# shenwei356/LexicMap

Measured on AMD Instinct MI355X. Metric: queries/sec (lexicmap search hot path, seed index HBM-resident), higher is better.
Workload: dtype u64

## Files before the change

### lexicmap_amd/csrc/lm_algos.h

```cpp
#pragma once
#include <stdint.h>

#if defined(__HIPCC__)
#define LM_HD __host__ __device__ __forceinline__
#define LM_HDN __host__ __device__ inline
#else
#define LM_HD inline
#define LM_HDN inline
#endif

#define LM_NULL_OFF (-1073741824)

LM_HD int lm_clz64(uint64_t x) {
#if defined(__HIP_DEVICE_COMPILE__)
    return x ? __clzll((long long)x) : 64;
#else
    return x ? __builtin_clzll(x) : 64;
#endif
}

LM_HD uint8_t lm_base2bit(uint8_t c) {
    switch (c | 0x20) {
    case 'c': case 'b': case 's': case 'y': return 1;
    case 'g': case 'k': return 2;
// ... 1165 lines not shown
    if ((key >> sh) & 3ull) return false;
    return lm_tree_search_miss(keys, n, key, p, K, lo, lo_out, hi_out);
}

#define LM_PFX_BASES 11
#define LM_PFX_BASES2 9
#define LM_PA_BLOOM_LOG_MAX 19
#define LM_PA_MAP9_LOG 18
LM_HD uint32_t lm_pa_filter_slot(uint32_t pfx, int log) {
    return (pfx * 0x9E3779B1u) >> (32 - log);
}
LM_HD int lm_pa_bloom_log(int log) { return log < LM_PA_BLOOM_LOG_MAX ? log : LM_PA_BLOOM_LOG_MAX; }
LM_HD uint32_t lm_mul24(uint32_t a, uint32_t b) {
#if defined(__HIP_DEVICE_COMPILE__)
    return __umul24(a, b);
#else
    return (uint32_t)((uint64_t)(a & 0xffffffu) * (uint64_t)(b & 0xffffffu));
#endif
}
LM_HD uint32_t lm_pa_bloom_slot(uint32_t pfx, int which, int blog) {
    return lm_mul24(pfx, which ? 0xB2AE35u : 0xEBCA6Bu) >> (32 - blog);
}
LM_HD uint64_t lm_pa_bits_words(int log) {
    return 2 * ((uint64_t)1 << (log - 5)) + ((uint64_t)1 << (lm_pa_bloom_log(log) - 5)) + ((uint64_t)1 << (LM_PA_MAP9_LOG - 5));
}
LM_HD int lm_pa_filter_log(int64_t nk) {
    int lg = 13;
    while (lg < 24 && ((int64_t)1 << lg) < 16 * nk) lg++;
    return lg;
}
#define LM_TAB_BITS_MIN 12
#define LM_TAB_BITS_MAX 20
LM_HD int lm_cmp_tab_bits(int64_t nk) {
    int tb = LM_TAB_BITS_MIN;
    while (tb < LM_TAB_BITS_MAX && ((int64_t)1 << tb) < 2 * nk) tb++;
    return tb;
}
LM_HD uint64_t lm_pa_bloom_word0(int log) { return 2 * ((uint64_t)1 << (log - 5)); }
LM_HD uint64_t lm_pa_map9_word0(int log) { return lm_pa_bloom_word0(log) + ((uint64_t)1 << (lm_pa_bloom_log(log) - 5)); }
template <typename OrBit> LM_HD void lm_pa_filter_set(uint64_t key, int K, int log, OrBit or_bit) {
    const uint32_t p11 = (uint32_t)(key >> ((K - LM_PFX_BASES) << 1)), p9 = (uint32_t)(key >> ((K - LM_PFX_BASES2) << 1));
    const int blog = lm_pa_bloom_log(log);
    const uint32_t h = lm_pa_filter_slot(p11, log), h2 = lm_pa_filter_slot(p9, log);
    or_bit((uint64_t)(h >> 5), 1u << (h & 31));
    or_bit(((uint64_t)1 << (log - 5)) + (h2 >> 5), 1u << (h2 & 31));
    const uint32_t a = lm_pa_bloom_slot(p11, 0, blog), b = lm_pa_bloom_slot(p11, 1, blog);
    or_bit(lm_pa_bloom_word0(log) + (a >> 5), 1u << (a & 31));
    or_bit(lm_pa_bloom_word0(log) + (b >> 5), 1u << (b & 31));
    or_bit(lm_pa_map9_word0(log) + (p9 >> 5), 1u << (p9 & 31));
}
LM_HD bool lm_pa_candidate(const uint32_t *bits, int log, uint64_t key, int p, int K) {
    const uint32_t h = lm_pa_filter_slot((uint32_t)(key >> ((K - LM_PFX_BASES) << 1)), log);
    if ((bits[h >> 5] >> (h & 31)) & 1u) return true;
    const uint64_t first_p = key >> ((K - p) << 1);
    if (first_p & ((1ull << ((p - 9) << 1)) - 1ull)) return false;
    if ((first_p & ((1ull << ((p - 7) << 1)) - 1ull)) == 0) return true;
    const uint32_t h2 = lm_pa_filter_slot((uint32_t)(key >> ((K - LM_PFX_BASES2) << 1)), log);
    const uint32_t *bits2 = bits + ((uint64_t)1 << (log - 5));
    return ((bits2[h2 >> 5] >> (h2 & 31)) & 1u) != 0;
}
LM_HD bool lm_pa_candidate2(const uint32_t *bloom, int blog, const uint32_t *map9, const uint32_t *bits11, int log,
                            uint32_t f, int p) {
    const uint32_t p11 = f >> ((p - LM_PFX_BASES) << 1);
    const uint32_t a = lm_pa_bloom_slot(p11, 0, blog), b = lm_pa_bloom_slot(p11, 1, blog);
    bool hit = (((bloom[a >> 5] >> (a & 31)) & (bloom[b >> 5] >> (b & 31))) & 1u) != 0;
    if (hit && log > blog) {
        const uint32_t h = lm_pa_filter_slot(p11, log);
        hit = ((bits11[h >> 5] >> (h & 31)) & 1u) != 0;
    }
    if (hit) return true;
    if (f & ((1u << ((p - 9) << 1)) - 1u)) return false;
    if ((f & ((1u << ((p - 7) << 1)) - 1u)) == 0) return true;
    const uint32_t p9 = f >> ((p - LM_PFX_BASES2) << 1);
    const bool m9 = ((map9[p9 >> 5] >> (p9 & 31)) & 1u) != 0;
    if (!m9) return false;
    if (p9 & 3u) {
        for (uint32_t sib = 1; sib < 4; sib++) {
            const uint32_t x = p11 | sib, sa = lm_pa_bloom_slot(x, 0, blog), sb = lm_pa_bloom_slot(x, 1, blog);
            bool h = (((bloom[sa >> 5] >> (sa & 31)) & (bloom[sb >> 5] >> (sb & 31))) & 1u) != 0;
            if (h && log > blog) {
                const uint32_t hh = lm_pa_filter_slot(x, log);
                h = ((bits11[hh >> 5] >> (hh & 31)) & 1u) != 0;
            }
            if (h) return true;
        }
        return false;
    }
    return true;
}

LM_HD bool lm_tree_search_range_tab(const uint64_t *keys, int n, uint64_t key, int p, int K, const uint32_t *tab,
                                    int tab_bits, int *lo_out, int *hi_out) {
    if (n <= 0) return false;
    if (p > K) p = K;
    const int sh = (K - p) << 1;
    const uint64_t low = sh >= 64 ? ~0ull : ((1ull << sh) - 1);
    const uint64_t left = key & ~low, right = key | low;
    const uint32_t b = (uint32_t)(key >> ((K << 1) - tab_bits));
    int lo = lm_lower_bound_u64(keys, (int)tab[b], (int)tab[b + 1], left);
    int hi = lm_upper_bound_u64(keys, lo, (int)tab[b + 1], right);
    if (lo < hi) {
        *lo_out = lo;
        *hi_out = hi;
        return true;
    }
    if ((key >> sh) & 3ull) return false;
    return lm_tree_search_miss(keys, n, key, p, K, lo, lo_out, hi_out);
}

LM_HD int lm_tree_search_first_tab(const uint64_t *keys, int n, uint64_t key, int p, int K, const uint32_t *tab, int tab_bits,
                                   int *lo_out, int *hi_out, uint64_t *right_out) {
// ... 434 lines not shown
```

### lexicmap_amd/csrc/lm_internal.h

```cpp
#pragma once
#include <hip/hip_runtime.h>

#include <algorithm>
#include <atomic>
#include <chrono>
#include <cstdio>
#include <cstdlib>
#include <map>
#include <memory>
#include <deque>
#include <mutex>
#include <shared_mutex>
#include <stdexcept>
#include <string>
#include <unordered_map>
#include <vector>

#include "../../include/lexicmap_hip.h"
#include "lm_format.h"
#include "lm_kernels.h"

namespace lm {

struct HipError : std::runtime_error {
// ... 372 lines not shown
    bool placing = false;
    void begin(lm_index *ix, int64_t local_genomes, int64_t max_genome_len);
    void count(const uint16_t *mask, const uint64_t *kmer, const uint64_t *val, int64_t n);
    void end_count();
    void place(const uint16_t *mask, const uint64_t *kmer, const uint64_t *val, int64_t n);
    void finish();
};
void sp_dump_range(const lm_index *src, hipStream_t st, const std::vector<int64_t> &off, bool flat, int64_t s0, int64_t s1,
                   uint16_t *s_mask, uint64_t *s_kmer, uint64_t *s_val, const uint64_t *new_bg = nullptr,
                   unsigned long long *n_out = nullptr);
void lm_screen_capture(lm_index *ix, hipStream_t st, const uint8_t *d_ascii, const std::vector<int64_t> &src_off,
                       const std::vector<int32_t> &len, const std::vector<int32_t> &reg_off, const std::vector<int32_t> &reg_s,
                       const std::vector<int32_t> &reg_e, uint64_t *d_kmers);
}

#define LM_WFA_CLASSES 5
struct lm_tune {
    int wfa_first_nc[LM_WFA_CLASSES] = {2, 2, 4, 8, 8};
    int wfa_win[LM_WFA_CLASSES] = {0, 0, 1, 0, 1};
    int chain1_wave = 1;
    int pa_filter_roll = 1;
    int pa_seg_by_group = 1;
    int pa_drop_nested = 1;
    int wfa_resident_pct = 100;
    int arena_reserve_pct = 90;
    int two_lanes = 1;
    int lookup_flat = 1;
    int wfa_r16 = 1;
    int wfa_serial = 0;
    int no_pipeline = 0;
    lm_tune() {
        if (const char *e = getenv("LM_WFA_FIRST_NC")) {
            int v[LM_WFA_CLASSES];
            if (sscanf(e, "%d,%d,%d,%d,%d", &v[0], &v[1], &v[2], &v[3], &v[4]) == LM_WFA_CLASSES)
                for (int c = 0; c < LM_WFA_CLASSES; c++)
                    if (v[c] == 1 || v[c] == 2 || v[c] == 4 || v[c] == 8 || v[c] == 16) wfa_first_nc[c] = v[c];
        }
        if (const char *e = getenv("LM_WFA_WIN"))
            for (int c = 0; c < LM_WFA_CLASSES && e[c]; c++) wfa_win[c] = e[c] == '1';
        if (const char *e = getenv("LM_WFA_R16")) wfa_r16 = atoi(e) != 0;
        if (const char *e = getenv("LM_LOOKUP_FLAT")) lookup_flat = atoi(e) != 0;
        if (const char *e = getenv("LM_CHAIN1_WAVE")) chain1_wave = atoi(e) != 0;
        if (const char *e = getenv("LM_TWO_LANES")) two_lanes = atoi(e) != 0;
        if (const char *e = getenv("LM_ARENA_RESERVE_PCT")) arena_reserve_pct = std::max(0, std::min(100, atoi(e)));
        if (const char *e = getenv("LM_PA_FILTER_ROLL")) pa_filter_roll = atoi(e) != 0;
        if (const char *e = getenv("LM_PA_DROP_NESTED")) pa_drop_nested = atoi(e) != 0;
    }
};

struct lm_index {
    lm_tune tune;
    int active_lanes = 1;
    int budget_lanes = 1;
    std::mutex mu;
    HostIndex host;
    lm_options opt;
    int device = 0;
    std::string err;
    DBuf<uint64_t> d_masks, d_pk_keys, d_pk_vals, d_out_kmers, d_out_vals, d_g_bg;
    DBuf<uint32_t> d_part_tab, d_g_keep;
    DBuf<int32_t> d_pfx_first, d_g_len, d_g2local;
    DBuf<int64_t> d_md_off, d_out_off, d_g_off, d_batch_first;
    int64_t n_seeds = 0, n_seeds_outlier = 0, seed_bytes = 0;
    int64_t scratch_budget = 0;
    DBuf<uint8_t> d_gbits;
    DBuf<float> d_gap_lut;
    int gap_lut_n = 0;
    DevIndexView view;
    int64_t hbm_bytes = 0;
// ... 48 lines not shown
```

### lexicmap_amd/csrc/lm_kernels.h

```cpp
#pragma once
#include <hip/hip_runtime.h>
#include <stdint.h>

#include "lm_algos.h"
#include "lm_residency.h"

namespace lm {

struct DevIndexView {
    int K, M, mask_prefix;
    const uint64_t *masks;
    const int32_t *pfx_first;
    int part_bases;
    int P1;
    int key_bits;
    int gid_bits, pos_bits;
    const uint64_t *pk_keys;
    const uint64_t *pk_vals;
    const uint32_t *part_tab;
    const int64_t *md_off;
    const uint64_t *g_bg;
    const uint32_t *g_keep;
    const uint64_t *out_kmers;
    const uint64_t *out_vals;
// ... 83 lines not shown
                       float min_score, int32_t *ntask);
void launch_make_tasks(hipStream_t st, DevIndexView ix, const uint64_t *segA, const int64_t *seg_off, int nseg,
                       const LmSub *subs, const int32_t *chain_off_pool, const int32_t *chain_idx_pool,
                       const int32_t *ntask, const int64_t *task_off, const int64_t *qoff, int ext_len,
                       int32_t *order_scratch, Task *tasks);
void launch_task_wlen(hipStream_t st, const Task *tasks, int64_t ntasks, int32_t *wlen);
void launch_task_set_woff(hipStream_t st, Task *tasks, int64_t ntasks, const int64_t *woff);
void launch_extract_windows(hipStream_t st, DevIndexView ix, const Task *tasks, const TaskSrc *src, int64_t ntasks,
                            const int32_t *only, uint8_t *wbuf);
void launch_extract_windows_at(hipStream_t st, DevIndexView ix, const Task *tasks, const TaskSrc *src, const int32_t *idx,
                               const int64_t *dest, int64_t n, uint8_t *wbuf);
void launch_stage_genome_bits(hipStream_t st, const StageCmd *cmds, int64_t n);
void launch_build_cmp_tab(hipStream_t st, const uint64_t *keys_cmp, const int64_t *posoff, const int32_t *nvalid, int nq,
                          int K, const int64_t *tab_off, const int32_t *tab_bits, int64_t tab_words, uint32_t *tab);
void launch_sum_i32(hipStream_t st, const int32_t *v, int64_t n, unsigned long long *out);
void launch_build_cmp_bits(hipStream_t st, const uint64_t *keys_cmp, const int64_t *posoff, const int32_t *nvalid, int nq,
                           int K, const int64_t *bits_off, const int32_t *bits_log, uint32_t *bits);
#define LM_PA_MAX_SEGS 8192
#define LM_PA_RANGE_SEGS 16
#define LM_PA_GROUP 64
void launch_pa_filter(hipStream_t st, DevIndexView ix, const Task *tasks, const TaskSrc *src, int64_t ntasks, const uint8_t *wbuf,
                      const int64_t *posoff, const int32_t *nvalid, const uint32_t *cmp_bits, const int64_t *bits_off,
                      const int32_t *bits_log, int K, int min_prefix, unsigned long long *seg_count, int nseg, int64_t seg_cap,
                      uint64_t *cand, unsigned long long *group_counter, int ncu, int seg_by_group, bool roll = true);
void launch_pa_search(hipStream_t st, DevIndexView ix, const Task *tasks, const TaskSrc *src, const uint8_t *wbuf, const uint64_t *keys_cmp,
                      const uint32_t *vals_cmp, const int64_t *posoff, const int32_t *nvalid, const uint32_t *cmp_tab,
                      const int64_t *tab_off, const int32_t *tab_bits, int K, int min_prefix,
                      const unsigned long long *seg_count, int nseg, int64_t seg_cap, const uint64_t *cand,
                      unsigned long long *count, int64_t cap, uint64_t *outA, uint64_t *outB, int qbits, int tbits,
                      int xcd_map, bool drop_nested = true);
void launch_pa_task_off_sorted(hipStream_t st, const uint64_t *sortedA, int shift, int64_t total, int64_t ntasks,
                               int64_t *pa_off);
void launch_pa_chain(hipStream_t st, const uint64_t *B, const int64_t *pa_off, int64_t ntasks, int K, LmChain2Opt opt,
                     LmSub *subs, uint8_t *marks, uint64_t *msi, int32_t *stack, LmChain2 *out, int32_t *out_n,
                     int32_t *clr_n, int qbits, int tbits);
void launch_gather_chain2(hipStream_t st, const LmChain2 *in, const int64_t *pa_off, const int32_t *out_n,
                          const int64_t *res_off, int64_t ntasks, LmChain2 *out);
void launch_extend_count(hipStream_t st, const HspIn *hsps, int64_t n, const uint8_t *qseq, const int64_t *qoff,
                         const uint8_t *wbuf, int32_t *cap);
void launch_extend_wave_cap(hipStream_t st, const int32_t *cap, int64_t n, int32_t *wcap, int64_t nw);
int extend_grid_blocks(int64_t n);
void launch_extend(hipStream_t st, const HspIn *hsps, int64_t n, const uint8_t *qseq, const int64_t *qoff,
                   const uint8_t *wbuf, const int32_t *cap, const int64_t *woff, uint16_t *subs, int32_t *msi,
                   void *rows_pool, uint32_t *rstart_pool, HspExt *out);
int wfa_resident_blocks(int device, int seq_words, int nc, bool win, bool r16 = false);
bool wfa_r16_ok(int seq_words, int nc, bool win);
void launch_wfa(hipStream_t st, const WfaIn *in, int64_t n, const int32_t *todo, int64_t ntodo, int nblocks,
// ... 9 lines not shown
```

### lexicmap_amd/csrc/lm_kernels.hip

```cpp
#include <hip/hip_runtime.h>
#include <stdint.h>

#include <algorithm>

#include "lm_algos.h"
#include "lm_kernels.h"
#include "lm_lookup_dev.h"

namespace lm {

#define LDS_WAVE_SYNC()                                        \
    do {                                                       \
        __builtin_amdgcn_fence(__ATOMIC_RELEASE, "wavefront"); \
        __builtin_amdgcn_wave_barrier();                       \
        __builtin_amdgcn_fence(__ATOMIC_ACQUIRE, "wavefront"); \
    } while (0)

__device__ __forceinline__ int find_segment(const int64_t *off, int n, int64_t x) {
    int lo = 0, hi = n;
    while (lo < hi) {
        int mid = (lo + hi + 1) >> 1;
        if (off[mid] <= x)
            lo = mid;
        else
// ... 63 lines not shown
        const int q = find_segment(tab_off, nq, t);
        const int bits = tab_bits[q], nb = 1 << bits;
        const int b = (int)(t - tab_off[q]);
        const uint64_t *keys = keys_cmp + 2 * posoff[q];
        int n = nvalid[q];
        int lo = n;
        if (b < nb) {
            uint64_t target = (uint64_t)b << ((K << 1) - bits);
            lo = lm_lower_bound_u64(keys, 0, n, target);
        }
        tab[t] = (uint32_t)lo;
    }
}
__global__ __launch_bounds__(256) void k_build_cmp_bits(const uint64_t *__restrict__ keys_cmp,
                                                         const int64_t *__restrict__ posoff,
                                                         const int32_t *__restrict__ nvalid, int nq, int K,
                                                         const int64_t *__restrict__ bits_off,
                                                         const int32_t *__restrict__ bits_log, uint32_t *__restrict__ bits) {
    for (int q = blockIdx.x; q < nq; q += gridDim.x) {
        const uint64_t *keys = keys_cmp + 2 * posoff[q];
        const int n = nvalid[q];
        const int log = bits_log[q];
        uint32_t *b = bits + bits_off[q];
        for (int j = threadIdx.x; j < n; j += blockDim.x)
            lm_pa_filter_set(keys[j], K, log, [&](uint64_t w, uint32_t m) { atomicOr(&b[w], m); });
    }
}

__global__ void k_fill_u32(uint32_t *p, int64_t n, uint32_t v) {
    for (int64_t i = (int64_t)blockIdx.x * blockDim.x + threadIdx.x; i < n; i += (int64_t)gridDim.x * blockDim.x) p[i] = v;
}

__global__ void k_mask(const uint64_t *__restrict__ keys_all, const int64_t *__restrict__ posoff, int nq, int M, int K,
                       const uint64_t *__restrict__ masks, uint64_t *__restrict__ out_kmers,
                       int64_t *__restrict__ out_lo, int64_t *__restrict__ out_hi, uint32_t *__restrict__ first_mask) {
    int64_t total = (int64_t)nq * M;
    for (int64_t t = (int64_t)blockIdx.x * blockDim.x + threadIdx.x; t < total; t += (int64_t)gridDim.x * blockDim.x) {
        int q = (int)(t / M), m = (int)(t % M);
        int64_t base = 2 * posoff[q];
        int n = (int)(2 * (posoff[q + 1] - posoff[q]));
        uint64_t kmer = 0;
        int lo = 0, hi = 0;
        if (n > 0) {
            kmer = lm_xor_argmin(keys_all + base, n, masks[m], &lo, &hi);
            if (kmer != 0 && lm_low_complexity(kmer, K)) kmer = 0;
            if (kmer != 0) atomicMin(&first_mask[base + lo], (uint32_t)m);
// ... 791 lines not shown
#define PA_SLICE_ROLL 2048
__device__ __forceinline__ uint32_t pa_rc16(uint32_t x) {
    const uint32_t y = __builtin_bitreverse32(~x);
    return ((y >> 1) & 0x55555555u) | ((y & 0x55555555u) << 1);
}
__device__ __forceinline__ bool pa_partial_rule(bool q, bool c, uint32_t f, int p, int blog, const uint32_t *bloom, const uint32_t *map9) {
    const uint32_t p9 = f >> ((p - 9) << 1);
    const bool all7 = (f & ((1u << ((p - 7) << 1)) - 1u)) == 0;
    const bool m9 = q && ((map9[p9 >> 5] >> (p9 & 31)) & 1u) != 0;
    const bool need = m9 && !all7 && (p9 & 3u) != 0;
    bool r = q ? (all7 || (m9 && (p9 & 3u) == 0)) : c;
    if (__ballot(need) != 0ull && need) {
        const uint32_t p11 = f >> ((p - LM_PFX_BASES) << 1);
        bool any = false;
#pragma unroll
        for (uint32_t sib = 1; sib < 4; sib++) {
            const uint32_t x = p11 | sib, sa = lm_pa_bloom_slot(x, 0, blog), sb = lm_pa_bloom_slot(x, 1, blog);
            any = any || (((bloom[sa >> 5] >> (sa & 31)) & (bloom[sb >> 5] >> (sb & 31))) & 1u) != 0;
        }
        r = any;
    }
    return r;
}
template <bool ROLL, bool SRC>
__global__ __launch_bounds__(PA_THREADS) void k_pa_filter(DevIndexView ix, const Task *__restrict__ tasks,
                                                           const TaskSrc *__restrict__ src, int64_t ntasks,
                                                           const uint8_t *__restrict__ wbuf,
                                                           const int64_t *__restrict__ posoff,
                                                           const int32_t *__restrict__ nvalid,
                                                           const uint32_t *__restrict__ cmp_bits,
                                                           const int64_t *__restrict__ bits_off,
                                                           const int32_t *__restrict__ bits_log, int K, int min_prefix,
                                                           unsigned long long *__restrict__ seg_count, int nseg,
                                                           int64_t seg_cap, uint64_t *__restrict__ cand,
                                                           unsigned long long *__restrict__ group_counter, int seg_by_group) {
    extern __shared__ uint64_t pa_lds[];
    uint64_t *s_stage = pa_lds;
    uint32_t *s_bloom = (uint32_t *)(pa_lds + PA_WAVES * PA_STAGE);
    uint32_t *s_map9 = s_bloom + (1 << (LM_PA_BLOOM_LOG_MAX - 5));
    uint64_t *s_pend_rec = (uint64_t *)(s_map9 + (1 << (LM_PA_MAP9_LOG - 5)));
    uint32_t *s_pend_pf = (uint32_t *)(s_pend_rec + PA_WAVES * PA_PEND);
    const int tid = threadIdx.x, lane = tid & 63, wave = tid >> 6;
    uint64_t *stg = s_stage + wave * PA_STAGE;
    int n_stg = 0;
    const uint64_t lt_mask = lane ? (~0ull >> (64 - lane)) : 0ull;
    int seg = (int)(((int64_t)blockIdx.x * PA_WAVES + wave) % nseg);
    uint64_t *seg_list = cand + (int64_t)seg * seg_cap;
// ... 5 lines not shown
        for (int j = lane; j < n_stg; j += 64)
            if ((int64_t)(base + (unsigned long long)j) < seg_cap) seg_list[base + (unsigned long long)j] = stg[j];
        n_stg = 0;
    };
    auto push = [&](bool c, uint64_t rec) {
        const uint64_t m = __ballot(c);
        if (m == 0) return;
        if (c) stg[n_stg + __popcll(m & lt_mask)] = rec;
        n_stg += __popcll(m);
        if (n_stg > PA_STAGE - 128) flush();
    };
    uint32_t *pend_pf = s_pend_pf + wave * PA_PEND;
    uint64_t *pend_rec = s_pend_rec + wave * PA_PEND;
    int n_pend = 0;
    const uint32_t *cur_qbits = nullptr;
    int cur_log = 0, cur_blog = 0;
    auto pend_round = [&](int cnt) {
        const int idx = n_pend - cnt + lane;
        bool c = false;
        uint64_t rec = 0;
        if (lane < cnt) {
            const uint32_t e = pend_pf[idx];
            rec = pend_rec[idx];
            c = lm_pa_candidate2(s_bloom, cur_blog, s_map9, cur_qbits, cur_log, e & 0x3fffffffu, LM_PFX_BASES + 2 * (int)(e >> 30));
        }
        n_pend -= cnt;
        push(c, rec);
    };
    auto pend = [&](bool c, uint32_t e, uint64_t rec) {
        const uint64_t m = __ballot(c);
        if (m == 0) return;
        if (c) {
            const int slot = n_pend + __popcll(m & lt_mask);
            pend_pf[slot] = e;
            pend_rec[slot] = rec;
        }
        n_pend += __popcll(m);
        while (n_pend >= 64) pend_round(64);
    };
    __shared__ int32_t s_q[PA_GROUP], s_rc[PA_GROUP], s_tb[PA_GROUP], s_wlen[PA_GROUP], s_npos[PA_GROUP], s_log[PA_GROUP];
    __shared__ int32_t s_first[PA_GROUP + 1];
    __shared__ int64_t s_goff[PA_GROUP], s_bits[PA_GROUP], s_woff[PA_GROUP];
    __shared__ const uint8_t *s_gb[SRC ? PA_GROUP : 1];
    __shared__ int s_next;
    __shared__ unsigned long long s_grp;
    const int64_t ngroups = (ntasks + PA_GROUP - 1) / PA_GROUP;
    while (true) {
        __syncthreads();
        if (tid == 0) s_grp = atomicAdd(group_counter, 1ull);
        __syncthreads();
        const int64_t grp = (int64_t)s_grp;
        if (grp >= ngroups) break;
        const int64_t t0g = grp * PA_GROUP;
        const int ng = (int)((ntasks < t0g + PA_GROUP ? ntasks : t0g + PA_GROUP) - t0g);
        if (seg_by_group) {
            const int gseg = (int)(grp * (int64_t)(nseg / PA_WAVES) / ngroups) * PA_WAVES + wave;
            if (gseg != seg) {
                flush();
                seg = gseg;
                seg_list = cand + (int64_t)seg * seg_cap;
// ... 9 lines not shown
            s_wlen[tid] = t.wlen;
            s_npos[tid] = n > 0 && t.wlen - K + 1 > 0 ? t.wlen - K + 1 : 0;
            if constexpr (SRC) {
                s_gb[tid] = t.g >= 0 ? src[t0g + tid].base : nullptr;
                s_goff[tid] = t.g >= 0 ? src[t0g + tid].off : 0;
            } else {
                s_goff[tid] = t.g >= 0 ? ix.g_off[t.g] : -1;
            }
            s_woff[tid] = t.woff;
            s_bits[tid] = cmp_bits ? bits_off[t.q] : -1;
            s_log[tid] = cmp_bits ? bits_log[t.q] : 0;
        }
        __syncthreads();
        int r0 = 0;
        while (r0 < ng) {
            int r1 = r0 + 1;
            while (r1 < ng && s_q[r1] == s_q[r0]) r1++;
            const int log = s_log[r0], blog = lm_pa_bloom_log(log);
            const uint32_t *qbits = s_bits[r0] >= 0 ? cmp_bits + s_bits[r0] : nullptr;
            cur_qbits = qbits;
            cur_log = log;
            cur_blog = blog;
            if (qbits != nullptr && K >= 16) {
                const uint32_t *gbl = qbits + lm_pa_bloom_word0(log), *g9 = qbits + lm_pa_map9_word0(log);
                const int nb = 1 << (blog - 5);
                for (int j = tid; j < nb; j += PA_THREADS) s_bloom[j] = gbl[j];
                for (int j = tid; j < (1 << (LM_PA_MAP9_LOG - 5)); j += PA_THREADS) s_map9[j] = g9[j];
            }
            if (tid == 0) {
                int acc = 0;
                for (int j = r0; j < r1; j++) {
                    s_first[j] = acc;
                    acc += (s_npos[j] + (ROLL ? PA_SLICE_ROLL : PA_SLICE) - 1) / (ROLL ? PA_SLICE_ROLL : PA_SLICE);
                }
                s_first[r1] = acc;
                s_next = 0;
            }
            __syncthreads();
            const int nslices = s_first[r1];
            while (true) {
                int sl = 0;
                if (lane == 0) sl = atomicAdd(&s_next, 1);
                sl = __builtin_amdgcn_readfirstlane(sl);
                if (sl >= nslices) break;
                int lo = r0, hi = r1;
                while (hi - lo > 1) {
                    const int mid = (lo + hi) >> 1;
// ... 46 lines not shown
#pragma unroll 1
                    for (int half = 0; half < 2; half++) {
#pragma unroll
                        for (int jj = 0; jj < 16; jj++) {
                            if (16 * half + jj >= bpl) break;
                            const int sh = 2 * jj;
                            const uint32_t xw = sh ? __builtin_amdgcn_alignbit(S0, S1, 32 - sh) : S0;
                            const int orc = 66 - 2 * jj;
                            const uint32_t Ra = (orc >> 5) == 2 ? R2 : R1, Rb = (orc >> 5) == 2 ? R3 : R2;
                            const uint32_t yw = (orc & 31) ? __builtin_amdgcn_alignbit(Ra, Rb, 32 - (orc & 31)) : Ra;
                            const uint32_t first = xw >> shp, rl = yw >> shp;
                            const uint32_t pf0 = t.rc ? rl : first, pf1 = t.rc ? first : rl;
                            const int r = rl0 + 16 * half + jj;
                            const int i = t.rc ? p1 - 1 - r : p0 + r;
                            const bool in = r < np;
                            bool c0, c1;
                            const uint32_t a0 = pf0 >> sha, a1 = pf1 >> sha;
                            const uint32_t s00 = lm_pa_bloom_slot(a0, 0, blog), s01 = lm_pa_bloom_slot(a0, 1, blog);
                            const uint32_t s10 = lm_pa_bloom_slot(a1, 0, blog), s11 = lm_pa_bloom_slot(a1, 1, blog);
                            const uint32_t b00 = s_bloom[s00 >> 5], b01 = s_bloom[s01 >> 5];
                            const uint32_t b10 = s_bloom[s10 >> 5], b11 = s_bloom[s11 >> 5];
                            const bool h0 = in && (((b00 >> (s00 & 31)) & (b01 >> (s01 & 31))) & 1u) != 0;
                            const bool h1 = in && (((b10 >> (s10 & 31)) & (b11 >> (s11 & 31))) & 1u) != 0;
                            const bool q0 = in && !h0 && (pf0 & m9p) == 0, q1 = in && !h1 && (pf1 & m9p) == 0;
                            c0 = h0;
                            c1 = h1;
                            if (log > blog) {
                                c0 = c1 = false;
                                const uint64_t rec = rec_t | ((uint64_t)(uint32_t)i << 1);
                                pend(h0 || q0, pf0 | pcode, rec);
                                pend(h1 || q1, pf1 | pcode, rec | 1ull);
                            } else if (__ballot(q0 || q1) != 0ull) {
                                c0 = pa_partial_rule(q0, c0, pf0, p, blog, s_bloom, s_map9);
                                c1 = pa_partial_rule(q1, c1, pf1, p, blog, s_bloom, s_map9);
                            }
                            const uint64_t m0 = __ballot(c0), m1 = __ballot(c1);
                            if ((m0 | m1) != 0ull) {
                                const int n0 = __popcll(m0);
                                const uint64_t rec = rec_t | ((uint64_t)(uint32_t)i << 1);
                                if (c0) stg[n_stg + __popcll(m0 & lt_mask)] = rec;
                                if (c1) stg[n_stg + n0 + __popcll(m1 & lt_mask)] = rec | 1ull;
                                n_stg += n0 + __popcll(m1);
                                if (n_stg > PA_STAGE - 128) flush();
                            }
                        }
                        S0 = S1;
                        S1 = S2;
                        R3 = R2;
                        R2 = R1;
                        R1 = R0;
                    }
                } else if (fast_pfx) {
                    const int np = p1 - p0;
                    const int g0 = t.rc ? t.tBegin + t.wlen - K - (p1 - 1) : t.tBegin + p0;
                    const int64_t abs0 = goff * 4 + g0;
                    const int64_t w0 = abs0 >> 5;
                    const int nwords = (int)(((abs0 + np + K - 2) >> 5) - w0) + 2;
                    const int lw = lane < nwords ? lane : nwords - 1;
                    const uint64_t Wl = __builtin_bswap64(((const uint64_t *)gb)[w0 + lw]);
                    for (int tile = 0; tile < np; tile += 64) {
                        const int r = tile + lane;
                        const int64_t ab = abs0 + r;
                        const int wi = (int)((ab >> 5) - w0), o = (int)(ab & 31) * 2;
                        const uint64_t H = __shfl(Wl, wi, 64), L = __shfl(Wl, wi + 1, 64);
                        const uint64_t v = o ? ((H << o) | (L >> (64 - o))) : H;
                        const uint32_t first = (uint32_t)(v >> (64 - 2 * p));
                        const uint32_t last = (uint32_t)(v >> (64 - 2 * K)) & ((1u << (2 * p)) - 1u);
                        const uint32_t rl = revcomp_small(last, p);
                        const uint32_t pf0 = t.rc ? rl : first, pf1 = t.rc ? first : rl;
                        const int i = t.rc ? p1 - 1 - r : p0 + r;
                        const bool in = r < np;
                        bool c0, c1;
                        {
                            const uint32_t a0 = pf0 >> ((p - LM_PFX_BASES) << 1), a1 = pf1 >> ((p - LM_PFX_BASES) << 1);
                            const uint32_t s00 = lm_pa_bloom_slot(a0, 0, blog), s01 = lm_pa_bloom_slot(a0, 1, blog);
                            const uint32_t s10 = lm_pa_bloom_slot(a1, 0, blog), s11 = lm_pa_bloom_slot(a1, 1, blog);
                            const uint32_t b00 = s_bloom[s00 >> 5], b01 = s_bloom[s01 >> 5];
                            const uint32_t b10 = s_bloom[s10 >> 5], b11 = s_bloom[s11 >> 5];
                            const bool h0 = in && (((b00 >> (s00 & 31)) & (b01 >> (s01 & 31))) & 1u) != 0;
                            const bool h1 = in && (((b10 >> (s10 & 31)) & (b11 >> (s11 & 31))) & 1u) != 0;
                            const uint32_t m9p = (1u << ((p - 9) << 1)) - 1u;
                            const bool q0 = in && !h0 && (pf0 & m9p) == 0, q1 = in && !h1 && (pf1 & m9p) == 0;
                            c0 = h0;
                            c1 = h1;
                            if (log > blog) {
                                c0 = c1 = false;
                                const uint64_t rec = rec_t | ((uint64_t)(uint32_t)i << 1);
                                const uint32_t pcode = (uint32_t)((p - LM_PFX_BASES) >> 1) << 30;
                                pend(h0 || q0, pf0 | pcode, rec);
                                pend(h1 || q1, pf1 | pcode, rec | 1ull);
                            } else if (__ballot(q0 || q1) != 0ull) {
                                c0 = pa_partial_rule(q0, c0, pf0, p, blog, s_bloom, s_map9);
                                c1 = pa_partial_rule(q1, c1, pf1, p, blog, s_bloom, s_map9);
                            }
                        }
                        const uint64_t m0 = __ballot(c0), m1 = __ballot(c1);
                        if ((m0 | m1) != 0ull) {
                            const int n0 = __popcll(m0);
                            const uint64_t rec = rec_t | ((uint64_t)(uint32_t)i << 1);
                            if (c0) stg[n_stg + __popcll(m0 & lt_mask)] = rec;
                            if (c1) stg[n_stg + n0 + __popcll(m1 & lt_mask)] = rec | 1ull;
                            n_stg += n0 + __popcll(m1);
                            if (n_stg > PA_STAGE - 128) flush();
                        }
                    }
                } else {
                    for (int tile = p0; tile < p1; tile += 64) {
                        const int i = tile + lane;
                        uint64_t kmer = 0, rc = 0;
                        if (i < p1) pa_kmer(t, w, gb, goff, i, K, &kmer, &rc);
#pragma unroll
                        for (int strand = 0; strand < 2; strand++) {
                            const bool c = i < p1 && (!use_bits || lm_pa_candidate(qbits, log, strand ? rc : kmer, p, K));
                            push(c, rec_t | ((uint64_t)(uint32_t)i << 1) | (uint64_t)strand);
                        }
                    }
// ... 1131 lines not shown
                               const int64_t *dest, int64_t n, uint8_t *wbuf) {
    if (n <= 0) return;
    hipLaunchKernelGGL(src ? k_extract_windows_at<true> : k_extract_windows_at<false>, dim3((unsigned)std::min<int64_t>(n, 65536)), dim3(256), 0, st, ix, tasks, src, idx, dest,
                       n, wbuf);
}
void launch_stage_genome_bits(hipStream_t st, const StageCmd *cmds, int64_t n) {
    if (n <= 0) return;
    hipLaunchKernelGGL(k_stage_genome_bits, dim3((unsigned)std::min<int64_t>(n, 65536)), dim3(256), 0, st, cmds, n);
}
void launch_build_cmp_tab(hipStream_t st, const uint64_t *keys_cmp, const int64_t *posoff, const int32_t *nvalid, int nq,
                          int K, const int64_t *tab_off, const int32_t *tab_bits, int64_t tab_words, uint32_t *tab) {
    LM_LAUNCH_1D(k_build_cmp_tab, tab_words, st, keys_cmp, posoff, nvalid, nq, K, tab_off, tab_bits, tab);
}
void launch_sum_i32(hipStream_t st, const int32_t *v, int64_t n, unsigned long long *out) {
    int g = (int)((n + 255) / 256);
    g = g < 1 ? 1 : (g > 2048 ? 2048 : g);
    hipLaunchKernelGGL(k_sum_i32, dim3(g), dim3(256), 0, st, v, n, out);
}
void launch_build_cmp_bits(hipStream_t st, const uint64_t *keys_cmp, const int64_t *posoff, const int32_t *nvalid, int nq,
                           int K, const int64_t *bits_off, const int32_t *bits_log, uint32_t *bits) {
    int g = nq < 1 ? 1 : (nq > 65536 ? 65536 : nq);
    hipLaunchKernelGGL(k_build_cmp_bits, dim3(g), dim3(256), 0, st, keys_cmp, posoff, nvalid, nq, K, bits_off, bits_log, bits);
}
void launch_pa_filter(hipStream_t st, DevIndexView ix, const Task *tasks, const TaskSrc *src, int64_t ntasks, const uint8_t *wbuf,
                      const int64_t *posoff, const int32_t *nvalid, const uint32_t *cmp_bits, const int64_t *bits_off,
                      const int32_t *bits_log, int K, int min_prefix, unsigned long long *seg_count, int nseg, int64_t seg_cap,
                      uint64_t *cand, unsigned long long *group_counter, int ncu, int seg_by_group, bool roll) {
    const int64_t ngroups = (ntasks + PA_GROUP - 1) / PA_GROUP;
    int g = (int)(ngroups < 1 ? 1 : (ngroups > ncu ? ncu : ngroups));
    static bool lds_set = false;
    if (!lds_set) {
        (void)hipFuncSetAttribute((const void *)k_pa_filter<true, false>, hipFuncAttributeMaxDynamicSharedMemorySize, PA_LDS_BYTES);
        (void)hipFuncSetAttribute((const void *)k_pa_filter<false, false>, hipFuncAttributeMaxDynamicSharedMemorySize, PA_LDS_BYTES);
        (void)hipFuncSetAttribute((const void *)k_pa_filter<true, true>, hipFuncAttributeMaxDynamicSharedMemorySize, PA_LDS_BYTES);
        (void)hipFuncSetAttribute((const void *)k_pa_filter<false, true>, hipFuncAttributeMaxDynamicSharedMemorySize, PA_LDS_BYTES);
        lds_set = true;
    }
    roll = roll && K == 31;
    auto kern = src ? (roll ? k_pa_filter<true, true> : k_pa_filter<false, true>) : (roll ? k_pa_filter<true, false> : k_pa_filter<false, false>);
    hipLaunchKernelGGL(kern, dim3(g), dim3(PA_THREADS), PA_LDS_BYTES, st, ix, tasks, src, ntasks, wbuf,
                       posoff, nvalid, cmp_bits, bits_off, bits_log, K, min_prefix, seg_count, nseg, seg_cap, cand, group_counter,
                       seg_by_group);
}
void launch_pa_search(hipStream_t st, DevIndexView ix, const Task *tasks, const TaskSrc *src, const uint8_t *wbuf, const uint64_t *keys_cmp,
                      const uint32_t *vals_cmp, const int64_t *posoff, const int32_t *nvalid, const uint32_t *cmp_tab,
                      const int64_t *tab_off, const int32_t *tab_bits, int K, int min_prefix,
                      const unsigned long long *seg_count, int nseg, int64_t seg_cap, const uint64_t *cand,
                      unsigned long long *count, int64_t cap, uint64_t *outA, uint64_t *outB, int qbits, int tbits,
                      int xcd_map, bool drop_nested) {
    int bps = xcd_map ? 256 / LM_PA_RANGE_SEGS : (256 * 32 + nseg - 1) / nseg;
    const int64_t need = (seg_cap + 255) / 256;
    if (bps > need) bps = (int)(need < 1 ? 1 : need);
    const int nseg8 = xcd_map ? (nseg / LM_PA_RANGE_SEGS + 7) / 8 * 8 * LM_PA_RANGE_SEGS : nseg;
    static const bool ps_dbg = getenv("LM_DEBUG_PA_SEARCH") != nullptr;
    static unsigned long long *d_dbg = nullptr;
    if (ps_dbg && !d_dbg && hipMalloc((void **)&d_dbg, 8 * sizeof(unsigned long long)) != hipSuccess) d_dbg = nullptr;
    if (ps_dbg && d_dbg) (void)hipMemsetAsync(d_dbg, 0, 8 * sizeof(unsigned long long), st);
    hipLaunchKernelGGL(src ? k_pa_search<true> : k_pa_search<false>, dim3(nseg8 * bps), dim3(256), 0, st, ix, tasks, src, wbuf, keys_cmp, vals_cmp, posoff, nvalid, cmp_tab,
                       tab_off, tab_bits, K, min_prefix, seg_count, seg_cap, bps, cand, count, cap, outA, outB, qbits, tbits, nseg,
                       xcd_map, drop_nested ? 1 : 0, ps_dbg ? d_dbg : nullptr);
    if (ps_dbg && d_dbg) {
        unsigned long long h[8] = {0};
// ... 95 lines not shown
```

### lexicmap_amd/csrc/lm_pipeline.hip

```cpp
#include <hip/hip_runtime.h>

#include <algorithm>
#include <chrono>
#include <cmath>
#include <cstdio>
#include <cstdlib>
#include <malloc.h>
#include <cstring>
#include <map>
#include <mutex>
#include <optional>
#include <sys/stat.h>
#include <stdexcept>
#include <tuple>
#include <string>
#include <unordered_map>
#include <vector>

#include "../../include/lexicmap_hip.h"
#include "lm_format.h"
#include "lm_kernels.h"

#include "lm_internal.h"
#include "lm_prims.h"
// ... 1502 lines not shown

extern "C" lm_status lm_qbatch_upload(lm_index *ix, const lm_query *queries, size_t nq, lm_qbatch **out) {
    *out = nullptr;
    if (!ix) return LM_ERR_ARG;
    if (nq >= ((size_t)1 << 31)) {
        ix->err = "query batch too large; split the batch";
        return LM_ERR_ARG;
    }
    try {
        std::lock_guard<std::mutex> lock(ix->mu);
        HIPCHK(hipSetDevice(ix->device));
        int64_t max_pos, max_qm;
        part_limits(ix, &max_pos, &max_qm);
        const int K = ix->host.k, M = ix->host.M;
        std::vector<size_t> cuts{0};
        int64_t pos = 0, nqp = 0;
        for (size_t i = 0; i < nq; i++) {
            const int64_t np = std::max<int64_t>((int64_t)queries[i].len - K + 1, 0);
            if (np > max_pos) {
                ix->err = "a query of " + std::to_string(queries[i].len) + " bases exceeds what one pass can hold (" +
                          std::to_string(max_pos) + " k-mers)";
                return LM_ERR_ARG;
            }
            if (nqp > 0 && (pos + np > max_pos || (nqp + 1) * (int64_t)M > max_qm)) {
                cuts.push_back(i);
                pos = 0;
                nqp = 0;
            }
            pos += np;
            nqp++;
        }
        cuts.push_back(nq);
        if (cuts.size() == 2) {
            *out = upload_part(ix, queries, nq, 0);
            return LM_OK;
        }
        lm_qbatch *top = new lm_qbatch();
        top->ix = ix;
        top->nq = (int)nq;
        try {
            for (size_t c = 0; c + 1 < cuts.size(); c++)
                top->parts.push_back(upload_part(ix, queries + cuts[c], cuts[c + 1] - cuts[c], (uint32_t)cuts[c]));
        } catch (...) {
            delete top;
            throw;
        }
        for (auto *p : top->parts) {
// ... 234 lines not shown
        for (int q = 0; q < qb->nq; q++) maxq = std::max<int64_t>(maxq, qb->h_qoff[q + 1] - qb->h_qoff[q]);
        if (maxq < 8192) by_group = false;
    }
    bool nseg_stale = false;
    for (int attempt = 0;; attempt++) {
        if (!compact) a.A0.ensure((size_t)a.pa_cap);
        a.B0.ensure((size_t)a.pa_cap);
        a.B1.ensure((size_t)a.pa_cap);
        if (!by_group) {
            if (attempt == 0 || nseg_stale) nseg = (int)std::max<int64_t>(1, std::min<int64_t>(1024, a.pa_cap / 4096));
            nseg_stale = false;
        } else if (attempt == 0) {
            const int64_t ngroups = (nt + LM_PA_GROUP - 1) / LM_PA_GROUP;
            const int64_t ranges = std::max<int64_t>(1, std::min<int64_t>(std::min<int64_t>(LM_PA_MAX_SEGS / LM_PA_RANGE_SEGS, ngroups),
                                                                          a.pa_cap / 4096 / LM_PA_RANGE_SEGS));
            nseg = (int)ranges * LM_PA_RANGE_SEGS;
        }
        const int64_t seg_cap = a.pa_cap / nseg;
        HIPCHK(hipMemsetAsync(a.pa_count.p, 0, (size_t)(2 + nseg) * sizeof(unsigned long long), S(ix)));
        {
            Prof p(ix, "k_pa_filter", W);
            launch_pa_filter(S(ix), ix->view, tasks_d, src_d, nt, a.wb, qb->posoff_cmp(), a.w->nvalid.p, a.w->cmp_bits.p,
                             qb->d_bits_off.p, qb->d_bits_log.p, LM_CMP_K, 11, a.pa_count.p + 2, nseg, seg_cap, a.B1.p,
                             a.pa_count.p + 1, device_cus(ix->device), by_group ? 1 : 0, ix->tune.pa_filter_roll != 0);
        }
        {
            Prof p(ix, "k_pa_search");
            launch_pa_search(S(ix), ix->view, tasks_d, src_d, a.wb, a.w->k_cmp, a.w->v_cmp, qb->posoff_cmp(), a.w->nvalid.p,
                             a.w->cmp_tab.p, qb->d_tab_off.p, qb->d_tab_bits.p, LM_CMP_K, 11, a.pa_count.p + 2, nseg, seg_cap,
                             a.B1.p, a.pa_count.p, a.pa_cap, a.A0.p, a.B0.p, compact ? qbits : 0, compact ? tbits : 0,
                             by_group ? 1 : 0, ix->tune.pa_drop_nested != 0);
        }
        std::vector<unsigned long long> hv((size_t)2 + nseg);
        HIPCHK(hipMemcpyAsync(hv.data(), a.pa_count.p, hv.size() * sizeof(unsigned long long), hipMemcpyDeviceToHost, S(ix)));
        sync(ix);
        TP = (int64_t)hv[0];
        int64_t ncand = 0, seg_max = 0;
        for (int j = 0; j < nseg; j++) {
            ncand += (int64_t)hv[2 + j];
            seg_max = std::max<int64_t>(seg_max, (int64_t)hv[2 + j]);
        }
        {
            int64_t idx = 0;
            uint32_t prevq = 0xffffffffu;
            for (int64_t i = 0; i < nt; i++)
                if (ht[i].q != prevq) {
                    prevq = ht[i].q;
// ... 2327 lines not shown
```

Measured before the change: 1377.

## Precompute partial-prefix rule bitmap per query to simplify prefix filter

Adds a second 9-base bitmap per query, built alongside the filter bits, that precomputes the partial-prefix acceptance rule (the sibling check over 11-mer prefixes). The prefix filter kernel gets a RULE template variant that tests this bit directly instead of running the sibling bloom loop, and only pends bloom hits that the rule does not already accept. A new pend2 helper batches both lanes with one ballot pass. The cost is more per-query bitmap memory (about 32 KB extra), a preset pass in the bit-build kernel, and query-batch splitting that now accounts for the larger bitmap, which may yield more batches.

```diff
diff --git a/lexicmap_amd/csrc/lm_algos.h b/lexicmap_amd/csrc/lm_algos.h
--- a/lexicmap_amd/csrc/lm_algos.h
+++ b/lexicmap_amd/csrc/lm_algos.h
@@ -1211,7 +1211,7 @@
     return lm_mul24(pfx, which ? 0xB2AE35u : 0xEBCA6Bu) >> (32 - blog);
 }
 LM_HD uint64_t lm_pa_bits_words(int log) {
-    return 2 * ((uint64_t)1 << (log - 5)) + ((uint64_t)1 << (lm_pa_bloom_log(log) - 5)) + ((uint64_t)1 << (LM_PA_MAP9_LOG - 5));
+    return 2 * ((uint64_t)1 << (log - 5)) + ((uint64_t)1 << (lm_pa_bloom_log(log) - 5)) + 2 * ((uint64_t)1 << (LM_PA_MAP9_LOG - 5));
 }
 LM_HD int lm_pa_filter_log(int64_t nk) {
     int lg = 13;
@@ -1227,6 +1227,10 @@
 }
 LM_HD uint64_t lm_pa_bloom_word0(int log) { return 2 * ((uint64_t)1 << (log - 5)); }
 LM_HD uint64_t lm_pa_map9_word0(int log) { return lm_pa_bloom_word0(log) + ((uint64_t)1 << (lm_pa_bloom_log(log) - 5)); }
+LM_HD uint64_t lm_pa_rule_word0(int log) { return lm_pa_map9_word0(log) + ((uint64_t)1 << (LM_PA_MAP9_LOG - 5)); }
+template <typename OrBit> LM_HD void lm_pa_filter_preset(int log, int j0, int step, OrBit or_bit) {
+    for (int j = j0; j < (1 << (LM_PA_MAP9_LOG - 5)); j += step) or_bit(lm_pa_rule_word0(log) + (uint64_t)j, 0x00010001u);
+}
 template <typename OrBit> LM_HD void lm_pa_filter_set(uint64_t key, int K, int log, OrBit or_bit) {
     const uint32_t p11 = (uint32_t)(key >> ((K - LM_PFX_BASES) << 1)), p9 = (uint32_t)(key >> ((K - LM_PFX_BASES2) << 1));
     const int blog = lm_pa_bloom_log(log);
@@ -1237,6 +1241,7 @@
     or_bit(lm_pa_bloom_word0(log) + (a >> 5), 1u << (a & 31));
     or_bit(lm_pa_bloom_word0(log) + (b >> 5), 1u << (b & 31));
     or_bit(lm_pa_map9_word0(log) + (p9 >> 5), 1u << (p9 & 31));
+    if ((p9 & 3u) == 0 || ((p11 & 0xfu) >= 1u && (p11 & 0xfu) <= 3u)) or_bit(lm_pa_rule_word0(log) + (p9 >> 5), 1u << (p9 & 31));
 }
 LM_HD bool lm_pa_candidate(const uint32_t *bits, int log, uint64_t key, int p, int K) {
     const uint32_t h = lm_pa_filter_slot((uint32_t)(key >> ((K - LM_PFX_BASES) << 1)), log);
@@ -1276,6 +1281,21 @@
         return false;
     }
     return true;
+}
+LM_HD bool lm_pa_rule_bit(const uint32_t *rule, uint32_t f, int p) {
+    const uint32_t p9 = f >> ((p - LM_PFX_BASES2) << 1);
+    return (f & ((1u << ((p - 9) << 1)) - 1u)) == 0 && ((rule[p9 >> 5] >> (p9 & 31)) & 1u) != 0;
+}
+LM_HD bool lm_pa_candidate3(const uint32_t *bloom, int blog, const uint32_t *rule, const uint32_t *bits11, int log,
+                            uint32_t f, int p) {
+    const uint32_t p11 = f >> ((p - LM_PFX_BASES) << 1);
+    const uint32_t a = lm_pa_bloom_slot(p11, 0, blog), b = lm_pa_bloom_slot(p11, 1, blog);
+    bool hit = (((bloom[a >> 5] >> (a & 31)) & (bloom[b >> 5] >> (b & 31))) & 1u) != 0;
+    if (hit && log > blog) {
+        const uint32_t h = lm_pa_filter_slot(p11, log);
+        hit = ((bits11[h >> 5] >> (h & 31)) & 1u) != 0;
+    }
+    return hit || lm_pa_rule_bit(rule, f, p);
 }
 
 LM_HD bool lm_tree_search_range_tab(const uint64_t *keys, int n, uint64_t key, int p, int K, const uint32_t *tab,
diff --git a/lexicmap_amd/csrc/lm_internal.h b/lexicmap_amd/csrc/lm_internal.h
--- a/lexicmap_amd/csrc/lm_internal.h
+++ b/lexicmap_amd/csrc/lm_internal.h
@@ -418,6 +418,7 @@
     int pa_filter_roll = 1;
     int pa_seg_by_group = 1;
     int pa_drop_nested = 1;
+    int pa_rule_map = 1;
     int wfa_resident_pct = 100;
     int arena_reserve_pct = 90;
     int two_lanes = 1;
@@ -441,6 +442,7 @@
         if (const char *e = getenv("LM_ARENA_RESERVE_PCT")) arena_reserve_pct = std::max(0, std::min(100, atoi(e)));
         if (const char *e = getenv("LM_PA_FILTER_ROLL")) pa_filter_roll = atoi(e) != 0;
         if (const char *e = getenv("LM_PA_DROP_NESTED")) pa_drop_nested = atoi(e) != 0;
+        if (const char *e = getenv("LM_PA_RULE_MAP")) pa_rule_map = atoi(e) != 0;
     }
 };
 
diff --git a/lexicmap_amd/csrc/lm_kernels.h b/lexicmap_amd/csrc/lm_kernels.h
--- a/lexicmap_amd/csrc/lm_kernels.h
+++ b/lexicmap_amd/csrc/lm_kernels.h
@@ -129,7 +129,8 @@
 void launch_pa_filter(hipStream_t st, DevIndexView ix, const Task *tasks, const TaskSrc *src, int64_t ntasks, const uint8_t *wbuf,
                       const int64_t *posoff, const int32_t *nvalid, const uint32_t *cmp_bits, const int64_t *bits_off,
                       const int32_t *bits_log, int K, int min_prefix, unsigned long long *seg_count, int nseg, int64_t seg_cap,
-                      uint64_t *cand, unsigned long long *group_counter, int ncu, int seg_by_group, bool roll = true);
+                      uint64_t *cand, unsigned long long *group_counter, int ncu, int seg_by_group, bool roll = true,
+                      bool rule = true);
 void launch_pa_search(hipStream_t st, DevIndexView ix, const Task *tasks, const TaskSrc *src, const uint8_t *wbuf, const uint64_t *keys_cmp,
                       const uint32_t *vals_cmp, const int64_t *posoff, const int32_t *nvalid, const uint32_t *cmp_tab,
                       const int64_t *tab_off, const int32_t *tab_bits, int K, int min_prefix,
diff --git a/lexicmap_amd/csrc/lm_kernels.hip b/lexicmap_amd/csrc/lm_kernels.hip
--- a/lexicmap_amd/csrc/lm_kernels.hip
+++ b/lexicmap_amd/csrc/lm_kernels.hip
@@ -109,6 +109,7 @@
         const int n = nvalid[q];
         const int log = bits_log[q];
         uint32_t *b = bits + bits_off[q];
+        lm_pa_filter_preset(log, (int)threadIdx.x, (int)blockDim.x, [&](uint64_t w, uint32_t m) { atomicOr(&b[w], m); });
         for (int j = threadIdx.x; j < n; j += blockDim.x)
             lm_pa_filter_set(keys[j], K, log, [&](uint64_t w, uint32_t m) { atomicOr(&b[w], m); });
     }
@@ -946,7 +947,7 @@
     }
     return r;
 }
-template <bool ROLL, bool SRC>
+template <bool ROLL, bool SRC, bool RULE>
 __global__ __launch_bounds__(PA_THREADS) void k_pa_filter(DevIndexView ix, const Task *__restrict__ tasks,
                                                            const TaskSrc *__restrict__ src, int64_t ntasks,
                                                            const uint8_t *__restrict__ wbuf,
@@ -998,7 +999,12 @@
         if (lane < cnt) {
             const uint32_t e = pend_pf[idx];
             rec = pend_rec[idx];
-            c = lm_pa_candidate2(s_bloom, cur_blog, s_map9, cur_qbits, cur_log, e & 0x3fffffffu, LM_PFX_BASES + 2 * (int)(e >> 30));
+            if constexpr (RULE) {
+                const uint32_t h = lm_pa_filter_slot((e & 0x3fffffffu) >> (4 * (int)(e >> 30)), cur_log);
+                c = ((cur_qbits[h >> 5] >> (h & 31)) & 1u) != 0;
+            } else {
+                c = lm_pa_candidate2(s_bloom, cur_blog, s_map9, cur_qbits, cur_log, e & 0x3fffffffu, LM_PFX_BASES + 2 * (int)(e >> 30));
+            }
         }
         n_pend -= cnt;
         push(c, rec);
@@ -1012,6 +1018,24 @@
             pend_rec[slot] = rec;
         }
         n_pend += __popcll(m);
+        while (n_pend >= 64) pend_round(64);
+    };
+    auto pend2 = [&](bool a0, bool a1, uint32_t e0, uint32_t e1, uint64_t rec) {
+        const uint64_t m0 = __ballot(a0), m1 = __ballot(a1);
+        if ((m0 | m1) == 0ull) return;
+        const int n0 = __popcll(m0), n1 = __popcll(m1);
+        if (n_pend + n0 + n1 > PA_PEND) pend_round(n_pend);
+        if (a0) {
+            const int slot = n_pend + __popcll(m0 & lt_mask);
+            pend_pf[slot] = e0;
+            pend_rec[slot] = rec;
+        }
+        if (a1) {
+            const int slot = n_pend + n0 + __popcll(m1 & lt_mask);
+            pend_pf[slot] = e1;
+            pend_rec[slot] = rec | 1ull;
+        }
+        n_pend += n0 + n1;
         while (n_pend >= 64) pend_round(64);
     };
     __shared__ int32_t s_q[PA_GROUP], s_rc[PA_GROUP], s_tb[PA_GROUP], s_wlen[PA_GROUP], s_npos[PA_GROUP], s_log[PA_GROUP];
@@ -1067,7 +1091,7 @@
             cur_log = log;
             cur_blog = blog;
             if (qbits != nullptr && K >= 16) {
-                const uint32_t *gbl = qbits + lm_pa_bloom_word0(log), *g9 = qbits + lm_pa_map9_word0(log);
+                const uint32_t *gbl = qbits + lm_pa_bloom_word0(log), *g9 = qbits + (RULE ? lm_pa_rule_word0(log) : lm_pa_map9_word0(log));
                 const int nb = 1 << (blog - 5);
                 for (int j = tid; j < nb; j += PA_THREADS) s_bloom[j] = gbl[j];
                 for (int j = tid; j < (1 << (LM_PA_MAP9_LOG - 5)); j += PA_THREADS) s_map9[j] = g9[j];
@@ -1160,17 +1184,28 @@
                             const uint32_t b10 = s_bloom[s10 >> 5], b11 = s_bloom[s11 >> 5];
                             const bool h0 = in && (((b00 >> (s00 & 31)) & (b01 >> (s01 & 31))) & 1u) != 0;
                             const bool h1 = in && (((b10 >> (s10 & 31)) & (b11 >> (s11 & 31))) & 1u) != 0;
-                            const bool q0 = in && !h0 && (pf0 & m9p) == 0, q1 = in && !h1 && (pf1 & m9p) == 0;
-                            c0 = h0;
-                            c1 = h1;
-                            if (log > blog) {
-                                c0 = c1 = false;
-                                const uint64_t rec = rec_t | ((uint64_t)(uint32_t)i << 1);
-                                pend(h0 || q0, pf0 | pcode, rec);
-                                pend(h1 || q1, pf1 | pcode, rec | 1ull);
-                            } else if (__ballot(q0 || q1) != 0ull) {
-                                c0 = pa_partial_rule(q0, c0, pf0, p, blog, s_bloom, s_map9);
-                                c1 = pa_partial_rule(q1, c1, pf1, p, blog, s_bloom, s_map9);
+                            if constexpr (RULE) {
+                                const bool r0 = in && lm_pa_rule_bit(s_map9, pf0, p), r1 = in && lm_pa_rule_bit(s_map9, pf1, p);
+                                c0 = h0 || r0;
+                                c1 = h1 || r1;
+                                if (log > blog) {
+                                    c0 = r0;
+                                    c1 = r1;
+                                    pend2(h0 && !r0, h1 && !r1, pf0 | pcode, pf1 | pcode, rec_t | ((uint64_t)(uint32_t)i << 1));
+                                }
+                            } else {
+                                const bool q0 = in && !h0 && (pf0 & m9p) == 0, q1 = in && !h1 && (pf1 & m9p) == 0;
+                                c0 = h0;
+                                c1 = h1;
+                                if (log > blog) {
+                                    c0 = c1 = false;
+                                    const uint64_t rec = rec_t | ((uint64_t)(uint32_t)i << 1);
+                                    pend(h0 || q0, pf0 | pcode, rec);
+                                    pend(h1 || q1, pf1 | pcode, rec | 1ull);
+                                } else if (__ballot(q0 || q1) != 0ull) {
+                                    c0 = pa_partial_rule(q0, c0, pf0, p, blog, s_bloom, s_map9);
+                                    c1 = pa_partial_rule(q1, c1, pf1, p, blog, s_bloom, s_map9);
+                                }
                             }
                             const uint64_t m0 = __ballot(c0), m1 = __ballot(c1);
                             if ((m0 | m1) != 0ull) {
@@ -1217,19 +1252,31 @@
                             const uint32_t b10 = s_bloom[s10 >> 5], b11 = s_bloom[s11 >> 5];
                             const bool h0 = in && (((b00 >> (s00 & 31)) & (b01 >> (s01 & 31))) & 1u) != 0;
                             const bool h1 = in && (((b10 >> (s10 & 31)) & (b11 >> (s11 & 31))) & 1u) != 0;
-                            const uint32_t m9p = (1u << ((p - 9) << 1)) - 1u;
-                            const bool q0 = in && !h0 && (pf0 & m9p) == 0, q1 = in && !h1 && (pf1 & m9p) == 0;
-                            c0 = h0;
-                            c1 = h1;
-                            if (log > blog) {
-                                c0 = c1 = false;
-                                const uint64_t rec = rec_t | ((uint64_t)(uint32_t)i << 1);
+                            if constexpr (RULE) {
+                                const bool r0 = in && lm_pa_rule_bit(s_map9, pf0, p), r1 = in && lm_pa_rule_bit(s_map9, pf1, p);
                                 const uint32_t pcode = (uint32_t)((p - LM_PFX_BASES) >> 1) << 30;
-                                pend(h0 || q0, pf0 | pcode, rec);
-                                pend(h1 || q1, pf1 | pcode, rec | 1ull);
-                            } else if (__ballot(q0 || q1) != 0ull) {
-                                c0 = pa_partial_rule(q0, c0, pf0, p, blog, s_bloom, s_map9);
-                                c1 = pa_partial_rule(q1, c1, pf1, p, blog, s_bloom, s_map9);
+                                c0 = h0 || r0;
+                                c1 = h1 || r1;
+                                if (log > blog) {
+                                    c0 = r0;
+                                    c1 = r1;
+                                    pend2(h0 && !r0, h1 && !r1, pf0 | pcode, pf1 | pcode, rec_t | ((uint64_t)(uint32_t)i << 1));
+                                }
+                            } else {
+                                const uint32_t m9p = (1u << ((p - 9) << 1)) - 1u;
+                                const bool q0 = in && !h0 && (pf0 & m9p) == 0, q1 = in && !h1 && (pf1 & m9p) == 0;
+                                c0 = h0;
+                                c1 = h1;
+                                if (log > blog) {
+                                    c0 = c1 = false;
+                                    const uint64_t rec = rec_t | ((uint64_t)(uint32_t)i << 1);
+                                    const uint32_t pcode = (uint32_t)((p - LM_PFX_BASES) >> 1) << 30;
+                                    pend(h0 || q0, pf0 | pcode, rec);
+                                    pend(h1 || q1, pf1 | pcode, rec | 1ull);
+                                } else if (__ballot(q0 || q1) != 0ull) {
+                                    c0 = pa_partial_rule(q0, c0, pf0, p, blog, s_bloom, s_map9);
+                                    c1 = pa_partial_rule(q1, c1, pf1, p, blog, s_bloom, s_map9);
+                                }
                             }
                         }
                         const uint64_t m0 = __ballot(c0), m1 = __ballot(c1);
@@ -2407,22 +2454,23 @@
     int g = nq < 1 ? 1 : (nq > 65536 ? 65536 : nq);
     hipLaunchKernelGGL(k_build_cmp_bits, dim3(g), dim3(256), 0, st, keys_cmp, posoff, nvalid, nq, K, bits_off, bits_log, bits);
 }
+static decltype(&k_pa_filter<true, true, true>) pa_filter_kernel(bool roll, bool src, bool rule) {
+    if (rule) return src ? (roll ? k_pa_filter<true, true, true> : k_pa_filter<false, true, true>) : (roll ? k_pa_filter<true, false, true> : k_pa_filter<false, false, true>);
+    return src ? (roll ? k_pa_filter<true, true, false> : k_pa_filter<false, true, false>) : (roll ? k_pa_filter<true, false, false> : k_pa_filter<false, false, false>);
+}
 void launch_pa_filter(hipStream_t st, DevIndexView ix, const Task *tasks, const TaskSrc *src, int64_t ntasks, const uint8_t *wbuf,
                       const int64_t *posoff, const int32_t *nvalid, const uint32_t *cmp_bits, const int64_t *bits_off,
                       const int32_t *bits_log, int K, int min_prefix, unsigned long long *seg_count, int nseg, int64_t seg_cap,
-                      uint64_t *cand, unsigned long long *group_counter, int ncu, int seg_by_group, bool roll) {
+                      uint64_t *cand, unsigned long long *group_counter, int ncu, int seg_by_group, bool roll, bool rule) {
     const int64_t ngroups = (ntasks + PA_GROUP - 1) / PA_GROUP;
     int g = (int)(ngroups < 1 ? 1 : (ngroups > ncu ? ncu : ngroups));
     static bool lds_set = false;
     if (!lds_set) {
-        (void)hipFuncSetAttribute((const void *)k_pa_filter<true, false>, hipFuncAttributeMaxDynamicSharedMemorySize, PA_LDS_BYTES);
-        (void)hipFuncSetAttribute((const void *)k_pa_filter<false, false>, hipFuncAttributeMaxDynamicSharedMemorySize, PA_LDS_BYTES);
-        (void)hipFuncSetAttribute((const void *)k_pa_filter<true, true>, hipFuncAttributeMaxDynamicSharedMemorySize, PA_LDS_BYTES);
-        (void)hipFuncSetAttribute((const void *)k_pa_filter<false, true>, hipFuncAttributeMaxDynamicSharedMemorySize, PA_LDS_BYTES);
+        for (int v = 0; v < 8; v++) (void)hipFuncSetAttribute((const void *)pa_filter_kernel(v & 1, v & 2, v & 4), hipFuncAttributeMaxDynamicSharedMemorySize, PA_LDS_BYTES);
         lds_set = true;
     }
     roll = roll && K == 31;
-    auto kern = src ? (roll ? k_pa_filter<true, true> : k_pa_filter<false, true>) : (roll ? k_pa_filter<true, false> : k_pa_filter<false, false>);
+    auto kern = pa_filter_kernel(roll, src != nullptr, rule);
     hipLaunchKernelGGL(kern, dim3(g), dim3(PA_THREADS), PA_LDS_BYTES, st, ix, tasks, src, ntasks, wbuf,
                        posoff, nvalid, cmp_bits, bits_off, bits_log, K, min_prefix, seg_count, nseg, seg_cap, cand, group_counter,
                        seg_by_group);
diff --git a/lexicmap_amd/csrc/lm_pipeline.hip b/lexicmap_amd/csrc/lm_pipeline.hip
--- a/lexicmap_amd/csrc/lm_pipeline.hip
+++ b/lexicmap_amd/csrc/lm_pipeline.hip
@@ -1548,7 +1548,8 @@
                           std::to_string(max_pos) + " k-mers)";
                 return LM_ERR_ARG;
             }
-            if (nqp > 0 && (pos + np > max_pos || (nqp + 1) * (int64_t)M > max_qm)) {
+            const int64_t per_q = (int64_t)M + (2 * ((int64_t)1 << (LM_PA_MAP9_LOG - 3)) + 79) / 80;
+            if (nqp > 0 && (pos + np > max_pos || (nqp + 1) * per_q > max_qm)) {
                 cuts.push_back(i);
                 pos = 0;
                 nqp = 0;
@@ -1829,7 +1830,8 @@
             Prof p(ix, "k_pa_filter", W);
             launch_pa_filter(S(ix), ix->view, tasks_d, src_d, nt, a.wb, qb->posoff_cmp(), a.w->nvalid.p, a.w->cmp_bits.p,
                              qb->d_bits_off.p, qb->d_bits_log.p, LM_CMP_K, 11, a.pa_count.p + 2, nseg, seg_cap, a.B1.p,
-                             a.pa_count.p + 1, device_cus(ix->device), by_group ? 1 : 0, ix->tune.pa_filter_roll != 0);
+                             a.pa_count.p + 1, device_cus(ix->device), by_group ? 1 : 0, ix->tune.pa_filter_roll != 0,
+                             ix->tune.pa_rule_map != 0);
         }
         {
             Prof p(ix, "k_pa_search");
```

New measurement: 1406 (median of 6 runs). 2.1% higher.
